# faverogian/diffusion-classifier

Hardware: AMD Instinct MI355X
Metric: images classified/sec (node), CIFAR-10 10-class x 50-step ELBO scoring (higher is better)
Workload: dtype bf16; 1 GPU; cifar10-unet-10x50; classes=10, trials=50, forwards_per_image=500, input=uniform [-1,1], parallelism=single

## Files before the change

### diffusion-classifier_amd/_lib.py

```python
import ctypes as C
import os

_HERE = os.path.dirname(os.path.abspath(__file__))
LIB_PATH = os.environ.get("DCAMD_LIB") or os.path.join(_HERE, "libdcamd.so")

ABI_VERSION = 4
DC_F32, DC_BF16, DC_F16 = 0, 1, 2
ACT_NONE, ACT_SILU, ACT_GEGLU, ACT_GELU_TANH = 0, 1, 2, 3
OP_QSAMPLE, OP_SINUSOID, OP_IGEMM, OP_GROUPNORM, OP_LAYERNORM, OP_ATTENTION, OP_EPS_MSE, OP_TBLOCK_FRONT = 1, 2, 3, 4, 5, 6, 7, 8

i32, i64, u64, f32, vp = C.c_int32, C.c_int64, C.c_uint64, C.c_float, C.c_void_p


class QsampleParams(C.Structure):
    _fields_ = [("x", vp), ("eps", vp), ("alpha", vp), ("sigma", vp), ("img_of_bj", vp),
                ("out", vp), ("out_dtype", i32),
                ("n_bj", i32), ("C", i32), ("H", i32), ("W", i32), ("ld", i32), ("im2col", i32), ("patch", i32)]


class SinusoidParams(C.Structure):
    _fields_ = [("lam", vp), ("out", vp), ("n", i32), ("dim", i32), ("flip_sin_to_cos", i32), ("freq_shift", f32)]


class IgemmParams(C.Structure):
# ... 39 lines not shown
    _fields_ = [("x", vp), ("Wp", vp), ("bp", vp), ("ln_g", vp), ("ln_b", vp), ("Wqkv", vp), ("Wo", vp), ("bo", vp),
                ("rowvec", vp), ("rowvec_map", vp), ("out", vp),
                ("dtype", i32), ("n", i32), ("L", i32), ("C", i32), ("heads", i32), ("ldx", i32), ("ld_out", i32), ("rowvec_ld", i32),
                ("ln_eps", f32), ("scale", f32)]


class EpsMseParams(C.Structure):
    _fields_ = [("pred", vp), ("eps", vp), ("x", vp), ("alpha", vp), ("sigma", vp),
                ("bj_of_unit", vp), ("img_of_bj", vp), ("out_index", vp),
                ("out", vp), ("n_units", i32), ("C", i32), ("H", i32), ("W", i32), ("ld", i32), ("v_param", i32), ("patch", i32)]


class DdpmStepParams(C.Structure):
    _fields_ = [("z", vp), ("pred", vp), ("noise", vp), ("out", vp),
                ("n", i32), ("C", i32), ("H", i32), ("W", i32), ("ld", i32), ("patch", i32), ("v_param", i32),
                ("w", f32), ("alpha_t", f32), ("sigma_t", f32), ("alpha_s", f32), ("c", f32), ("sd", f32), ("one_plus_w", f32)]


class Op(C.Structure):
    _fields_ = [("kind", i32), ("pad_", i32), ("params", vp)]


EXPORTS = ["dc_abi_version", "dc_last_error", "dc_arch", "dc_qsample", "dc_philox_normal", "dc_sinusoid",
           "dc_igemm", "dc_igemm_cout_pad", "dc_igemm_variant", "dc_igemm_gn_fusable", "dc_igemm_side_ok", "dc_igemm_ln_ok", "dc_igemm_qstats_parts", "dc_igemm_up4_ok", "dc_igemm_pn_ok", "dc_pn_timeouts", "dc_groupnorm", "dc_groupnorm_variant", "dc_groupnorm_ws_floats", "dc_groupnorm_splits",
           "dc_layernorm", "dc_layernorm_variant", "dc_attention", "dc_attention_variant", "dc_tblock_front", "dc_tblock_front_ok", "dc_eps_mse", "dc_ddpm_step", "dc_haar_dwt2", "dc_haar_idwt2", "dc_stage_topk", "dc_reduce_argmin", "dc_stage_maps", "dc_run_plan", "dc_run_plan_timed",
           "dc_packed_bytes", "dc_pack_weights_matrix", "dc_pack_weights_conv3x3", "dc_pack_weights_up4", "dc_pack_weights_geglu",
           "dc_fold_layernorm_bias", "dc_workspace_bytes_groupnorm", "dc_workspace_bytes_igemm", "dc_workspace_bytes_attention",
           "dc_workspace_bytes_layernorm"]

_lib = None


class DcamdError(RuntimeError):
    pass


def lib():
    global _lib
    if _lib is not None:
        return _lib
    if not os.path.exists(LIB_PATH):
        raise DcamdError(
            f"HIP extension {LIB_PATH} is missing — build it with `python -c 'import __graft_entry__ as g; g.build()'` "
            "(or `make -C diffusion-classifier_amd/csrc`). There is no CPU fallback for the scoring path.")
    L = C.CDLL(LIB_PATH)
    L.dc_abi_version.restype = i32
    L.dc_last_error.restype = C.c_char_p
# ... 19 lines not shown
                       ("dc_fold_layernorm_bias", [vp, vp, vp, i32, i32, vp, vp]),
                       ("dc_stage_topk", [vp, i32, i32, i32, i32, i32, vp, vp, vp]),
                       ("dc_reduce_argmin", [vp, i32, i32, i32, i32, vp, vp, vp]),
                       ("dc_stage_maps", [vp, i32, i32, i32, i32, i32, i32, i32, i32, i32, i32, i32, vp, vp])]:
        fn = getattr(L, name)
        fn.argtypes = argt
        fn.restype = i32
    L.dc_igemm_ln_ok.argtypes = [C.POINTER(IgemmParams)]
    L.dc_igemm_ln_ok.restype = C.c_int32
    L.dc_igemm_qstats_parts.argtypes = [C.POINTER(IgemmParams)]
    L.dc_igemm_qstats_parts.restype = C.c_int32
    L.dc_igemm_up4_ok.argtypes = [C.POINTER(IgemmParams)]
    L.dc_igemm_up4_ok.restype = C.c_int32
    L.dc_igemm_pn_ok.argtypes = [C.POINTER(IgemmParams)]
    L.dc_igemm_pn_ok.restype = C.c_int32
    L.dc_tblock_front_ok.argtypes = [C.POINTER(TblockFrontParams)]
    L.dc_tblock_front_ok.restype = C.c_int32
    L.dc_pn_timeouts.argtypes = []
    L.dc_pn_timeouts.restype = C.c_int32
    L.dc_igemm_side_ok.argtypes = [C.POINTER(IgemmParams)]
    L.dc_igemm_side_ok.restype = C.c_int32
    L.dc_igemm_variant.argtypes = [C.POINTER(IgemmParams)]
    L.dc_igemm_variant.restype = C.c_char_p
    L.dc_attention_variant.argtypes = [C.POINTER(AttentionParams)]
    L.dc_attention_variant.restype = C.c_char_p
    L.dc_groupnorm_variant.argtypes = [C.POINTER(GroupnormParams)]
    L.dc_groupnorm_variant.restype = C.c_char_p
    L.dc_layernorm_variant.argtypes = [C.POINTER(LayernormParams)]
    L.dc_layernorm_variant.restype = C.c_char_p
    L.dc_igemm_gn_fusable.argtypes = [C.POINTER(IgemmParams)]
    L.dc_igemm_gn_fusable.restype = i32
    L.dc_igemm_cout_pad.argtypes = [i32, i32]
    L.dc_igemm_cout_pad.restype = i32
    L.dc_packed_bytes.argtypes = [i32, i32, i32, i32]
    L.dc_packed_bytes.restype = i64
    for name, pt in (("dc_workspace_bytes_groupnorm", GroupnormParams), ("dc_workspace_bytes_igemm", IgemmParams),
                     ("dc_workspace_bytes_attention", AttentionParams), ("dc_workspace_bytes_layernorm", LayernormParams)):
        getattr(L, name).argtypes = [C.POINTER(pt)]
        getattr(L, name).restype = i64
    L.dc_groupnorm_ws_floats.argtypes = [i32, i32, i32]
    L.dc_groupnorm_ws_floats.restype = i64
    L.dc_groupnorm_splits.argtypes = [i32, i32, i32]
    L.dc_groupnorm_splits.restype = i32
    if L.dc_abi_version() != ABI_VERSION:
        raise DcamdError(f"libdcamd ABI {L.dc_abi_version()} != {ABI_VERSION} (stale libdcamd.so? rebuild with `make -C diffusion-classifier_amd/csrc`)")
    _lib = L
# ... 19 lines not shown
```

### diffusion-classifier_amd/csrc/igemm.hip

```cpp
#include <stdio.h>
#include <stdlib.h>
#include "conv3_halo.h"

template <typename T, int BM, int BN, int WGM, int WGN>
__global__ __launch_bounds__(256, 2) void igemm_kernel(const IgemmArgs a) {
  constexpr int EPC = Elem<T>::EPC;
  constexpr int BKE = 8 * EPC;
  constexpr int XL = BM / 32;
  constexpr int WL = (BN + 31) / 32;
  constexpr int WTM = BM / WGM, WTN = BN / WGN;
  constexpr int TM = WTM / 16, TN = WTN / 16;
  static_assert(WGM * WGN == 4, "4 waves");
  extern __shared__ __attribute__((aligned(16))) char smem[];
  constexpr int BUF = (BM + BN) * 128;

  const int t = threadIdx.x;
  const int lane = t & 63, wave = t >> 6;
  const int wm = wave / WGN, wn = wave % WGN;
  const int lr = lane & 15, lq = lane >> 4;

  int tile_m, tile_n;
  tile_of_block(a, tile_m, tile_n);

  const int HWo = a.Hout * a.Wout;
// ... 282 lines not shown
    case IG_PIPE: return dc_igemm_launch_pipe(a, p->dtype, c.shape, s);
    case IG_REG128: return dc_by_dtype(p->dtype, "dc_igemm: dtype", [&](auto t) { return launch<decltype(t), 128, 128, 2, 2>(a, s); });
    case IG_REG32: return dc_by_dtype(p->dtype, "dc_igemm: dtype", [&](auto t) { return launch<decltype(t), 128, 32, 4, 1>(a, s); });
  }
  return DC_ERR_ARG;
}

extern "C" int dc_igemm(const dc_igemm_params* p, dc_stream stream) {
  IgemmArgs a;
  const int rc = igemm_validate_and_fill(p, a);
  if (rc != DC_OK) return rc;
  const IgemmChoice c = igemm_choose(p, a);
  if (c.status != DC_OK) { dc_set_error("%s", c.message); return c.status; }
  return igemm_launch(c, a, p, stream);
}

extern "C" const char* dc_igemm_variant(const dc_igemm_params* p) {
  IgemmArgs a;
  if (igemm_validate_and_fill(p, a) != DC_OK) return "invalid";
  const IgemmChoice c = igemm_choose(p, a);
  return c.status == DC_OK ? igemm_name(c, p->dtype) : c.tag;
}

static int32_t igemm_accepts(const dc_igemm_params& q) {
  IgemmArgs a;
  return igemm_validate_and_fill(&q, a) == DC_OK && igemm_choose(&q, a).status == DC_OK ? 1 : 0;
}
alignas(16) static float g_probe_dummy[4] = {0.f, 0.f, 0.f, 0.f};

extern "C" int32_t dc_igemm_gn_fusable(const dc_igemm_params* p) {
  if (!p) return 0;
  dc_igemm_params q = *p;
  q.gn_scale = g_probe_dummy; q.gn_shift = g_probe_dummy;
  return igemm_accepts(q);
}

extern "C" int32_t dc_igemm_ln_ok(const dc_igemm_params* p) {
  if (!p) return 0;
  dc_igemm_params q = *p;
  if (!(q.ln_eps > 0.f)) q.ln_eps = 1e-5f;
  return igemm_accepts(q);
}

extern "C" int32_t dc_igemm_qstats_parts(const dc_igemm_params* p) {
  if (!p) return 0;
  dc_igemm_params q = *p;
// ... 35 lines not shown
```

### diffusion-classifier_amd/csrc/igemm_common.h

```cpp
#pragma once
#include "common.h"

struct IgemmArgs {
  const void* src0; const int32_t* map0; const void* src1; const int32_t* map1;
  const void* W; const float* bias;
  const float* rowvec; const int32_t* rowvec_map;
  const float* gate; const int32_t* gate_map;
  const void* residual; const int32_t* res_map;
  void* out;
  const float* gn_scale; const float* gn_shift; int gn_silu;
  const void* src2; const int32_t* map2; const void* W2; int C2, ld2;
  float ln_eps;
  float* qstats;
  void* pn_out; const float* pn_gamma; const float* pn_beta; unsigned* pn_cnt; int pn_ld, pn_groups, pn_silu; float pn_eps;
  int C0, C1, ld0, ld1, rowvec_ld, gate_ld, res_dtype, res_ld, out_dtype, out_ld, act;
  int taps, stride, upsample, Hin, Win, Hout, Wout, Cout;
  int M, Ktot, c0chunks, cpt, nk, tiles_m, tiles_n;
  int n_fast;
};

template <typename T> struct Mma;
template <> struct Mma<__bf16> {
  static __device__ __forceinline__ f32x4 run(const chunk16 w, const chunk16 x, f32x4 acc) {
    return __builtin_amdgcn_mfma_f32_16x16x32_bf16(__builtin_bit_cast(bf16x8, w), __builtin_bit_cast(bf16x8, x), acc, 0, 0, 0);
// ... 83 lines not shown
      }
      if (oc + 3 < cout_out && (a.out_ld & 3) == 0) {
        if (a.out_dtype == DC_F32) {
          *reinterpret_cast<float4*>(reinterpret_cast<float*>(a.out) + orow + oc) = make_float4(v[0], v[1], v[2], v[3]);
        } else if (a.out_dtype == DC_BF16) {
          __bf16 h[4] = {(__bf16)v[0], (__bf16)v[1], (__bf16)v[2], (__bf16)v[3]};
          *reinterpret_cast<uint2*>(reinterpret_cast<__bf16*>(a.out) + orow + oc) = *reinterpret_cast<uint2*>(h);
        } else {
          _Float16 h[4] = {(_Float16)v[0], (_Float16)v[1], (_Float16)v[2], (_Float16)v[3]};
          *reinterpret_cast<uint2*>(reinterpret_cast<_Float16*>(a.out) + orow + oc) = *reinterpret_cast<uint2*>(h);
        }
      } else {
#pragma unroll
        for (int r = 0; r < 4; ++r)
          if (oc + r < cout_out) store_as(a.out, orow + oc + r, a.out_dtype, v[r]);
      }
    }
  }
}

int dc_igemm_pipe_shape(const IgemmArgs& a);
int dc_igemm_launch_pipe(const IgemmArgs& a, int dtype, int shape, hipStream_t s);
int dc_igemm_launch_wide8(const IgemmArgs& a, int dtype, hipStream_t s);
__device__ __forceinline__ void tile_of_block_scalar(const IgemmArgs& a, int& tile_m, int& tile_n) {
  tile_of_block(a, tile_m, tile_n);
  tile_m = __builtin_amdgcn_readfirstlane(tile_m);
  tile_n = __builtin_amdgcn_readfirstlane(tile_n);
  asm volatile("" : "+s"(tile_m), "+s"(tile_n));
}

bool dc_conv3_halo_applicable(const IgemmArgs& a, int dtype);
int dc_conv3_halo_launch(const IgemmArgs& a, int dtype, int n_img, hipStream_t s);
bool dc_conv3_up4_applicable(const IgemmArgs& a, int dtype);
int dc_conv3_up4_launch(const IgemmArgs& a, int dtype, int n_img, hipStream_t s);
int dc_igemm_launch_pipe_up4(const IgemmArgs& a, int dtype, hipStream_t s);
bool dc_conv3_halo_pn_ok(const IgemmArgs& a, int dtype, bool up4);
unsigned dc_conv3_halo_pn_timeouts();
bool dc_conv3_ws_ok(const IgemmArgs& a, int dtype);
int dc_conv3_ws_launch(const IgemmArgs& a, int dtype, int n_img, hipStream_t s);
bool dc_igemm_xreg_applicable(const IgemmArgs& a, int dtype);
int dc_igemm_xreg_launch(const IgemmArgs& a, int dtype, hipStream_t s);
bool dc_conv3_thin_applicable(const IgemmArgs& a, int dtype);
int dc_conv3_thin_launch(const IgemmArgs& a, int dtype, int n_img, hipStream_t s);
```

### diffusion-classifier_amd/csrc/igemm_epilogue.h

```cpp
#pragma once
#include "igemm_common.h"
#ifndef DC_STAMP
#define DC_STAMP(k) do {} while (0)
#endif
#ifndef DC_HALO_ABL
#define DC_HALO_ABL() 0
#endif

__device__ __forceinline__ int epi_wrow(int R, bool geglu) {
  const int wn = R >> 6, i = (R >> 4) & 3, lq = (R >> 2) & 3, reg = R & 3;
  if (geglu) {
    const int o = wn * 32 + lq * 8 + (i >> 1) * 4 + reg;
    return (o >> 4) * 32 + ((i & 1) << 4) + (o & 15);
  }
  return wn * 64 + (i >> 1) * 32 + lq * 8 + (i & 1) * 4 + reg;
}

struct EpiRow { int o, r, samp; bool ok; };

__device__ __forceinline__ void ld8(const float* p, float (&v)[8]) {
  const f32x4 a = *reinterpret_cast<const f32x4*>(p), b = *reinterpret_cast<const f32x4*>(p + 4);
#pragma unroll
  for (int e = 0; e < 4; ++e) { v[e] = a[e]; v[4 + e] = b[e]; }
}

struct EpiNoPre { __device__ __forceinline__ void operator()() const {} };
struct EpiNoBias {
  static constexpr bool on = false, has_rowvec = false;
  __device__ __forceinline__ void operator()(int, float (&)[8], float (&)[8]) const {}
};

template <int V> struct EpiIC { static constexpr int value = V; };
struct EpiNoPnLocal { static constexpr bool on = false; static constexpr int IMG_FR = 4; };
struct EpiPnLocal8x8 { static constexpr bool on = true; static constexpr int IMG_FR = 4; };
struct EpiPnLocal4x4 { static constexpr bool on = true; static constexpr int IMG_FR = 1; };
struct EpiNoQs {
  static constexpr bool on = false;
  __device__ __forceinline__ bool operator()(int, int&, int&) const { return false; }
  __device__ __forceinline__ bool whole() const { return true; }
  __device__ __forceinline__ int parts() const { return 1; }
};

template <typename T, int TM, int ACT, bool GATE, bool TWO_SAMP, typename RowFn, typename PreFn = EpiNoPre, typename QsFn = EpiNoQs,
          typename BiasFn = EpiNoBias, typename PnL = EpiNoPnLocal>
__device__ __forceinline__ void epi_direct_act(const IgemmArgs& a, f32x4 (&acc)[4][TM], int tile_n, int wn, int lq,
                                               int samp_first, int samp_last, RowFn rowfn, PreFn prefn = PreFn(), QsFn qsfn = QsFn(),
                                               BiasFn biasfn = BiasFn(), PnL = PnL()) {
  static_assert(!PnL::on || (TM == 8 && ACT == DC_ACT_NONE && !GATE && (QsFn::on || PnL::IMG_FR == 1)), "wave-local GroupNorm: the plain 128-pixel halo epilogue");
  constexpr bool geglu = ACT == DC_ACT_GEGLU;
  constexpr int NK = geglu ? 1 : 2;
  constexpr int JB = TM;
  const int cout_out = geglu ? (a.Cout >> 1) : a.Cout;
  const int c0 = (geglu ? tile_n * 64 + wn * 32 : tile_n * 128 + wn * 64) + lq * 8;
  constexpr bool res16 = sizeof(T) == 2;
  bool con[NK];
#pragma unroll
  for (int k = 0; k < NK; ++k) con[k] = c0 + 32 * k < cout_out;

  {
    float bs[NK][8], bgt[8];
#pragma unroll
    for (int k = 0; k < NK; ++k) {
      const int c = c0 + 32 * k;
#pragma unroll
      for (int e = 0; e < 8; ++e) { bs[k][e] = 0.f; if (k == 0) bgt[e] = 0.f; }
      if constexpr (BiasFn::on) {
        biasfn(k, bs[k], bgt);
      } else if (a.bias && con[k]) {
        const int p = geglu ? (c >> 4) * 32 + (c & 15) : c;
        ld8(a.bias + p, bs[k]);
        if (geglu) ld8(a.bias + p + 16, bgt);
      }
    }
    const bool uni = samp_first == samp_last;
    prefn();
    const bool rv_uni = !BiasFn::has_rowvec && !geglu && a.rowvec && uni;
    float rvu[NK][8];
#pragma unroll
    for (int k = 0; k < NK; ++k)
#pragma unroll
      for (int e = 0; e < 8; ++e) rvu[k][e] = 0.f;
    if (rv_uni) {
#pragma unroll
      for (int k = 0; k < NK; ++k)
        if (con[k]) ld8(a.rowvec + (size_t)(a.rowvec_map ? a.rowvec_map[samp_first] : samp_first) * a.rowvec_ld + c0 + 32 * k, rvu[k]);
    }
#pragma unroll
    for (int j = 0; j < TM; ++j)
#pragma unroll
      for (int e = 0; e < 8; ++e) {
        if (geglu) { acc[(e >> 2) * 2][j][e & 3] += bs[0][e]; acc[(e >> 2) * 2 + 1][j][e & 3] += bgt[e]; }
        else {
#pragma unroll
          for (int k = 0; k < NK; ++k) acc[2 * k + (e >> 2)][j][e & 3] += bs[k][e];
        }
      }
    if (rv_uni) {
#pragma unroll
      for (int j = 0; j < TM; ++j)
#pragma unroll
        for (int e = 0; e < 8; ++e)
#pragma unroll
          for (int k = 0; k < NK; ++k) acc[2 * k + (e >> 2)][j][e & 3] += rvu[k][e];
    }
    if (!BiasFn::has_rowvec && !geglu && a.rowvec && !uni) {
      if (TWO_SAMP) {
#pragma unroll
        for (int k = 0; k < NK; ++k)
          if (con[k]) {
            float ra[8], rb[8];
            ld8(a.rowvec + (size_t)(a.rowvec_map ? a.rowvec_map[samp_first] : samp_first) * a.rowvec_ld + c0 + 32 * k, ra);
            ld8(a.rowvec + (size_t)(a.rowvec_map ? a.rowvec_map[samp_last] : samp_last) * a.rowvec_ld + c0 + 32 * k, rb);
#pragma unroll
            for (int j = 0; j < TM; ++j) {
              EpiRow rj;
              rowfn(j, rj);
              const bool second = rj.samp != samp_first;
#pragma unroll
              for (int e = 0; e < 8; ++e) acc[2 * k + (e >> 2)][j][e & 3] += second ? rb[e] : ra[e];
            }
          }
      } else {
#pragma unroll
        for (int j = 0; j < TM; ++j) {
          EpiRow rj;
          rowfn(j, rj);
#pragma unroll
          for (int k = 0; k < NK; ++k)
            if (con[k]) {
              float rv[8];
              ld8(a.rowvec + (size_t)(a.rowvec_map ? a.rowvec_map[rj.samp] : rj.samp) * a.rowvec_ld + c0 + 32 * k, rv);
#pragma unroll
              for (int e = 0; e < 8; ++e) acc[2 * k + (e >> 2)][j][e & 3] += rv[e];
            }
        }
      }
    }
  }

  DC_STAMP(3);
  int orow[TM];
#pragma unroll
  for (int j0 = 0; j0 < TM; j0 += JB) {
    EpiRow row[JB];
#pragma unroll
    for (int jj = 0; jj < JB; ++jj) { rowfn(j0 + jj, row[jj]); orow[j0 + jj] = row[jj].ok ? row[jj].o : -1; }
    chunk16 rc[JB][NK];
#pragma unroll
    for (int jj = 0; jj < JB; ++jj)
#pragma unroll
      for (int k = 0; k < NK; ++k) {
        rc[jj][k] = chunk16{0u, 0u, 0u, 0u};
        if (res16 && a.residual && row[jj].ok && con[k])
          rc[jj][k] = *reinterpret_cast<const chunk16*>(reinterpret_cast<const char*>(a.residual) + ((size_t)row[jj].r * a.res_ld + c0 + 32 * k) * 2);
      }
    if (j0 == 0) DC_STAMP(4);
#pragma unroll
    for (int jj = 0; jj < JB; ++jj) {
      const int j = j0 + jj;
#pragma unroll
      for (int k = 0; k < NK; ++k) {
        if (!(row[jj].ok && con[k])) continue;
        float rf[8], gt[8];
#pragma unroll
        for (int e = 0; e < 8; ++e) { rf[e] = 0.f; gt[e] = 1.f; }
        if (GATE) ld8(a.gate + (size_t)(a.gate_map ? a.gate_map[row[jj].samp] : row[jj].samp) * a.gate_ld + c0 + 32 * k, gt);
        if (a.residual) {
          if (!res16) ld8(reinterpret_cast<const float*>(a.residual) + (size_t)row[jj].r * a.res_ld + c0 + 32 * k, rf);
          else chunk_to_f<T>(rc[jj][k], rf);
        }
#pragma unroll
        for (int e = 0; e < 8; ++e) {
          if (geglu) {
            acc[(e >> 2) * 2][j][e & 3] = acc[(e >> 2) * 2][j][e & 3] * gelu_erf_t<T>(acc[(e >> 2) * 2 + 1][j][e & 3]) + rf[e];
          } else {
            float x = acc[2 * k + (e >> 2)][j][e & 3];
            if (ACT == DC_ACT_SILU) x = silu_t<T>(x);
            if (ACT == DC_ACT_GELU_TANH) x = gelu_tanh_t<T>(x);
            if (GATE) x *= gt[e];
            acc[2 * k + (e >> 2)][j][e & 3] = x + rf[e];
          }
        }
      }
    }
  }
  DC_STAMP(5);
  float pnr[(PnL::on && PnL::IMG_FR == 4) ? 2 : 1][NK][4];
  float pgm[PnL::on ? NK : 1][8], pbt[PnL::on ? NK : 1][8];
  if constexpr (PnL::on) {
#pragma unroll
// ... 47 lines not shown
            r[k][2 * qd] = __builtin_fmaf(S, inv_n, piv[k][qd]);
            r[k][2 * qd + 1] = fmaxf(__builtin_fmaf(-S * S, inv_n, Q), 0.f);
          }
        if constexpr (PnL::on && PnL::IMG_FR == 4) {
#pragma unroll
          for (int k = 0; k < NK; ++k)
#pragma unroll
            for (int e = 0; e < 4; ++e) pnr[h][k][e] = r[k][e];
        }
        int n = 0, part = 0;
        if ((threadIdx.x & 15) == 0 && qsfn(h, n, part)) {
#pragma unroll
          for (int k = 0; k < NK; ++k)
            if (con[k])
              *reinterpret_cast<f32x4*>(a.qstats + (((size_t)n * qsfn.parts() + part) * (a.Cout >> 2) + ((c0 + 32 * k) >> 2)) * 2) =
                  f32x4{r[k][0], r[k][1], r[k][2], r[k][3]};
        }
      };
      if (qsfn.whole()) emit(EpiIC<0>{}, EpiIC<TM>{}, 0);
      else { emit(EpiIC<0>{}, EpiIC<TM / 2>{}, 0); emit(EpiIC<TM / 2>{}, EpiIC<TM>{}, 1); }
    }
  }
  auto store_all = [&](void* outp, int ld, int odt) {
    if (odt == DC_F32) {
#pragma unroll
      for (int j = 0; j < TM; ++j)
#pragma unroll
        for (int k = 0; k < NK; ++k)
          if (orow[j] >= 0 && con[k]) {
            float* op = reinterpret_cast<float*>(outp) + (size_t)orow[j] * ld + c0 + 32 * k;
            if (geglu) { *reinterpret_cast<f32x4*>(op) = acc[0][j]; *reinterpret_cast<f32x4*>(op + 4) = acc[2][j]; }
            else { *reinterpret_cast<f32x4*>(op) = acc[2 * k][j]; *reinterpret_cast<f32x4*>(op + 4) = acc[2 * k + 1][j]; }
          }
    } else {
#pragma unroll
      for (int j = 0; j < TM; ++j)
#pragma unroll
        for (int k = 0; k < NK; ++k)
          if (orow[j] >= 0 && con[k]) {
            float v[8];
#pragma unroll
            for (int e = 0; e < 8; ++e) v[e] = geglu ? acc[(e >> 2) * 2][j][e & 3] : acc[2 * k + (e >> 2)][j][e & 3];
            *reinterpret_cast<chunk16*>(reinterpret_cast<T*>(outp) + (size_t)orow[j] * ld + c0 + 32 * k) = f_to_chunk<T>(v);
          }
    }
  };
  if constexpr (!PnL::on) {
    store_all(a.out, a.out_ld, a.out_dtype);
  } else {
    if (a.out) store_all(a.out, a.out_ld, a.out_dtype);
    constexpr int IFR = PnL::IMG_FR, NIMG = TM / IFR;
    const int qpg = (a.Cout / a.pn_groups) >> 2;
    const float nq = (float)(IFR * 64);
#pragma unroll
    for (int h = 0; h < NIMG; ++h) {
#pragma unroll
      for (int k = 0; k < NK; ++k) {
        float rq[4];
        if constexpr (IFR == 4) {
#pragma unroll
          for (int e = 0; e < 4; ++e) rq[e] = pnr[h][k][e];
        } else {
#pragma clang fp contract(off)
          auto share0l = [](float v) { return __builtin_bit_cast(float, __builtin_amdgcn_update_dpp(0, __builtin_bit_cast(int, v), 0x150, 0xF, 0xF, true)); };
          auto row_suml = [](float v) {
            v += __builtin_bit_cast(float, __builtin_amdgcn_update_dpp(0, __builtin_bit_cast(int, v), 0xB1, 0xF, 0xF, true));
            v += __builtin_bit_cast(float, __builtin_amdgcn_update_dpp(0, __builtin_bit_cast(int, v), 0x4E, 0xF, 0xF, true));
            v += __builtin_bit_cast(float, __builtin_amdgcn_update_dpp(0, __builtin_bit_cast(int, v), 0x141, 0xF, 0xF, true));
            v += __builtin_bit_cast(float, __builtin_amdgcn_update_dpp(0, __builtin_bit_cast(int, v), 0x140, 0xF, 0xF, true));
            return v;
          };
// ... 59 lines not shown
        if (a.pn_silu) {
#pragma unroll
          for (int jj = 0; jj < IFR; ++jj)
#pragma unroll
            for (int e = 0; e < 8; ++e) {
              const float x = acc[2 * k + (e >> 2)][h * IFR + jj][e & 3];
              acc[2 * k + (e >> 2)][h * IFR + jj][e & 3] = silu_t<T>(x * ga[e] + gb[e]);
            }
        } else {
#pragma unroll
          for (int jj = 0; jj < IFR; ++jj)
#pragma unroll
            for (int e = 0; e < 8; ++e) {
              const float x = acc[2 * k + (e >> 2)][h * IFR + jj][e & 3];
              acc[2 * k + (e >> 2)][h * IFR + jj][e & 3] = x * ga[e] + gb[e];
            }
        }
      }
    }
    store_all(a.pn_out, a.pn_ld, sizeof(T) == 4 ? DC_F32 : (int)a.out_dtype);
  }
}

template <typename T, int TM, typename RowFn>
__device__ __forceinline__ void epi_direct(const IgemmArgs& a, f32x4 (&acc)[4][TM], int tile_n, int wn, int lq,
                                           int samp_first, int samp_last, RowFn rowfn) {
  switch (a.act) {
    case DC_ACT_SILU: epi_direct_act<T, TM, DC_ACT_SILU, false, false>(a, acc, tile_n, wn, lq, samp_first, samp_last, rowfn); break;
    case DC_ACT_GEGLU: epi_direct_act<T, TM, DC_ACT_GEGLU, false, false>(a, acc, tile_n, wn, lq, samp_first, samp_last, rowfn); break;
    case DC_ACT_GELU_TANH: epi_direct_act<T, TM, DC_ACT_GELU_TANH, false, false>(a, acc, tile_n, wn, lq, samp_first, samp_last, rowfn); break;
    default:
      if (a.gate) epi_direct_act<T, TM, DC_ACT_NONE, true, false>(a, acc, tile_n, wn, lq, samp_first, samp_last, rowfn);
      else epi_direct_act<T, TM, DC_ACT_NONE, false, false>(a, acc, tile_n, wn, lq, samp_first, samp_last, rowfn);
      break;
  }
}
```

### diffusion-classifier_amd/csrc/igemm_wide.hip

```cpp
#include <stdlib.h>
#include "igemm_epilogue.h"

static __device__ chunk16 g_zero_page_w[16];
DC_CLOCK_DECL(igemm_wide)

typedef const __attribute__((address_space(1))) void* gptr_t;
typedef __attribute__((address_space(3))) void* lptr_t;

template <typename T, int EV>
__global__ __launch_bounds__(512, 2) void igemm_wide8_kernel(const IgemmArgs a) {
  constexpr int EPC = Elem<T>::EPC;
  constexpr int BKE = 8 * EPC;
  constexpr int HALF = 128 * 128;
  constexpr int BUF = 4 * HALF;
  constexpr int SX0 = 0, SW0 = HALF, SX1 = 2 * HALF, SW1 = 3 * HALF;
  extern __shared__ __attribute__((aligned(16))) char smem[];

  const int t = threadIdx.x;
  const int lane = t & 63;
  const int wave = __builtin_amdgcn_readfirstlane(t >> 6);
  const int wm = wave >> 1, wn = wave & 1;
  const int lr = lane & 15, lq = lane >> 4;
  int tile_m, tile_n;
  tile_of_block(a, tile_m, tile_n);
  const int HWo = a.Hout * a.Wout;
  const int nk = a.nk, c0chunks = a.c0chunks;

  const int lchunk = (t & 7) ^ ((t >> 4) & 7);
  const T* xr0[2][2]; const T* xr1[2][2];
  int wro[2][2];
#pragma unroll
  for (int i = 0; i < 2; ++i) {
    const int hr = 64 * i + (t >> 3);
#pragma unroll
    for (int xh = 0; xh < 2; ++xh) {
      const int m = tile_m * 256 + (hr >> 5) * 64 + xh * 32 + (hr & 31);
      const bool vm = m < a.M;
      const int mm = vm ? m : 0;
      const int n = mm / HWo;
      const int rem = mm - n * HWo;
      const int n0 = a.map0 ? a.map0[n] : n;
      const int n1 = a.src1 ? (a.map1 ? a.map1[n] : n) : 0;
      const T* b0 = reinterpret_cast<const T*>(a.src0) + ((size_t)n0 * HWo + rem) * a.ld0 + lchunk * EPC;
      const T* b1 = reinterpret_cast<const T*>(a.src1) + ((size_t)n1 * HWo + rem) * a.ld1 + lchunk * EPC;
      xr0[xh][i] = vm ? b0 : nullptr;
      xr1[xh][i] = (vm && a.src1) ? b1 : nullptr;
      asm volatile("" ::"v"(xr0[xh][i]), "v"(xr1[xh][i]));
// ... 57 lines not shown
  _Pragma("unroll") for (int sub = 0; sub < 2; ++sub)                                                         \
    _Pragma("unroll") for (int jj = 0; jj < 2; ++jj)                                                          \
      _Pragma("unroll") for (int i = 0; i < 4; ++i)                                                           \
        acc[H][i][J0 + jj] = Mma<T>::run(wf[sub][i], XF[sub][jj], acc[H][i][J0 + jj]);                        \
  __builtin_amdgcn_s_setprio(0);                                                                              \
  __builtin_amdgcn_sched_barrier(0);
#define W8_READ_X(DST, SLOT)                                                                                \
  _Pragma("unroll") for (int sub = 0; sub < 2; ++sub) {                                                       \
    DST[sub][0] = ds_read16_async_off<SLOT>(xfo[sub] + bufo);                                                 \
    DST[sub][1] = ds_read16_async_off<SLOT + 2048>(xfo[sub] + bufo);                                          \
  }
#define W8_READ_W(SLOT)                                                                                     \
  _Pragma("unroll") for (int sub = 0; sub < 2; ++sub) {                                                       \
    wf[sub][0] = ds_read16_async_off<SLOT>(wfo[sub] + bufo);                                                  \
    wf[sub][1] = ds_read16_async_off<SLOT + 2048>(wfo[sub] + bufo);                                           \
    wf[sub][2] = ds_read16_async_off<SLOT + 4096>(wfo[sub] + bufo);                                           \
    wf[sub][3] = ds_read16_async_off<SLOT + 6144>(wfo[sub] + bufo);                                           \
  }
#define W8_WAIT_W() asm volatile("s_waitcnt lgkmcnt(0)" : "+v"(wf[0][0]), "+v"(wf[0][1]), "+v"(wf[0][2]), "+v"(wf[0][3]), \
                                 "+v"(wf[1][0]), "+v"(wf[1][1]), "+v"(wf[1][2]), "+v"(wf[1][3]))
#define W8_WAIT_X(XF) asm volatile("s_waitcnt lgkmcnt(0)" : "+v"(XF[0][0]), "+v"(XF[0][1]), "+v"(XF[1][0]), "+v"(XF[1][1]))

  DC_CLOCK(0);
  for (int kt = 0; kt < nk; ++kt) {
    const uint32_t bufo = (uint32_t)(kt & 1) * BUF;
    lgkm_fence0();
    W8_READ_X(xa, SX0)
    __builtin_amdgcn_sched_barrier(0);
    W8_READ_W(SW0)
    stage_w(kt + 1, 1, SW1);
    asm volatile("s_waitcnt lgkmcnt(8)" : "+v"(xa[0][0]), "+v"(xa[0][1]), "+v"(xa[1][0]), "+v"(xa[1][1]));
    __builtin_amdgcn_s_barrier();
    W8_WAIT_W();
    W8_MMA(0, xa, 0)
    __builtin_amdgcn_s_barrier();
    W8_READ_X(xb, SX1)
    stage_x(kt + 2, 0, SX0);
    __builtin_amdgcn_s_barrier();
    W8_WAIT_X(xb);
    W8_MMA(0, xb, 2)
    __builtin_amdgcn_s_barrier();
    W8_READ_W(SW1)
    stage_w(kt + 2, 0, SW0);
    __builtin_amdgcn_s_barrier();
    W8_WAIT_W();
    W8_MMA(1, xb, 2)
    __builtin_amdgcn_s_barrier();
    stage_x(kt + 2, 1, SX1);
    if (kt + 2 < nk) asm volatile("s_waitcnt vmcnt(6)" ::: "memory");
    else asm volatile("s_waitcnt vmcnt(0)" ::: "memory");
    __builtin_amdgcn_s_barrier();
    W8_MMA(1, xa, 0)
    __builtin_amdgcn_s_barrier();
  }
#undef W8_MMA
#undef W8_READ_X
#undef W8_READ_W
#undef W8_WAIT_W
#undef W8_WAIT_X
  DC_CLOCK(1);
  if (wave < 4) __builtin_amdgcn_s_barrier();

  const int mw0 = tile_m * 256 + wm * 64;
  auto rowfn = [&](int j, EpiRow& r) {
    const int m = mw0 + j * 16 + lr;
    r.ok = m < a.M;
    const int mm = r.ok ? m : a.M - 1;
    const int n = mm / HWo;
    r.samp = n;
    r.o = mm;
    r.r = (a.residual && a.res_map) ? a.res_map[n] * HWo + (mm - n * HWo) : mm;
  };
  const int sf = min(mw0, a.M - 1) / HWo, sl = min(mw0 + 63, a.M - 1) / HWo;
  constexpr int ACT = EV == 3 ? DC_ACT_GELU_TANH : (EV == 2 ? DC_ACT_GEGLU : DC_ACT_NONE);
  epi_direct_act<T, 4, ACT, EV == 4, false>(a, acc[0], tile_n * 2 + wn, 0, lq, sf, sl, rowfn);
  __builtin_amdgcn_sched_barrier(0);
  epi_direct_act<T, 4, ACT, EV == 4, false>(a, acc[1], tile_n * 2 + wn, 1, lq, sf, sl, rowfn);
}

template <typename T, int EV>
static int launch_wide8(const IgemmArgs& a0, hipStream_t s) {
  constexpr int lds = 2 * 4 * 128 * 128;
  static bool attr_done = false;
  auto kern = igemm_wide8_kernel<T, EV>;
  if (!attr_done) {
    (void)hipFuncSetAttribute(reinterpret_cast<const void*>(kern), hipFuncAttributeMaxDynamicSharedMemorySize, lds);
    attr_done = true;
  }
  IgemmArgs a = a0;
  a.tiles_m = (a.M + 255) / 256;
  a.tiles_n = a0.tiles_n / 2;
  const long long nblk = (long long)a.tiles_m * a.tiles_n;
  if (nblk <= 0 || nblk > 0x7fffffffLL) { dc_set_error("dc_igemm: bad grid %lld", nblk); return DC_ERR_SHAPE; }
  if ((long long)a0.tiles_n * 128 * a.Ktot >= (1LL << 31)) { dc_set_error("dc_igemm(wide8): weight matrix of %d x %d too large", a0.tiles_n * 128, a.Ktot); return DC_ERR_SHAPE; }
  hipLaunchKernelGGL(kern, dim3((unsigned)nblk), dim3(512), lds, s, a);
  return dc_check_launch("dc_igemm(wide8)");
}

template <typename T>
static int launch_wide8_t(const IgemmArgs& a, hipStream_t s) {
  if (a.act == DC_ACT_GELU_TANH) return launch_wide8<T, 3>(a, s);
  if (a.act == DC_ACT_GEGLU) return launch_wide8<T, 2>(a, s);
  if (a.gate) return launch_wide8<T, 4>(a, s);
  return launch_wide8<T, 0>(a, s);
}

int dc_igemm_launch_wide8(const IgemmArgs& a, int dtype, hipStream_t s) {
  return dc_by_dtype(dtype, "dc_igemm: dtype", [&](auto t) { return launch_wide8_t<decltype(t)>(a, s); });
}
```

### include/dcamd.h

```cpp
#ifndef DCAMD_H
#define DCAMD_H

#include <stddef.h>
#include <stdint.h>

#ifdef __cplusplus
extern "C" {
#endif

#define DC_ABI_VERSION 4

typedef void* dc_stream;

typedef enum { DC_OK = 0, DC_ERR_ARG = -1, DC_ERR_SHAPE = -2, DC_ERR_DTYPE = -3,
               DC_ERR_ALIGN = -4, DC_ERR_LAUNCH = -5, DC_ERR_UNSUPPORTED = -6 } dc_status;

typedef enum { DC_F32 = 0, DC_BF16 = 1, DC_F16 = 2 } dc_dtype;

typedef enum { DC_ACT_NONE = 0, DC_ACT_SILU = 1, DC_ACT_GEGLU = 2, DC_ACT_GELU_TANH = 3 } dc_act;

int dc_abi_version(void);
const char* dc_last_error(void);
const char* dc_arch(void);

// ... 13 lines not shown

typedef struct {
  int32_t dtype, taps, stride, upsample;
  int32_t n_img, Hin, Win, Hout, Wout;
  const void* src0; const int32_t* map0; int32_t C0, ld0;
  const void* src1; const int32_t* map1; int32_t C1, ld1;
  const void* W; int32_t Cout, tile_n;
  const float* bias;
  const float* rowvec; const int32_t* rowvec_map; int32_t rowvec_ld, act;
  const float* gate; const int32_t* gate_map; int32_t gate_ld, pad2_;
  const void* residual; const int32_t* res_map; int32_t res_dtype, res_ld;
  void* out; int32_t out_dtype, out_ld;
  const float* gn_scale; const float* gn_shift; int32_t gn_silu, pad3_;
  const void* src2; const int32_t* map2; const void* W2; int32_t C2, ld2;
  float ln_eps;
  int32_t up4;
  float* qstats;
  void* pn_out; const float* pn_gamma; const float* pn_beta; uint32_t* pn_cnt;
  int32_t pn_ld, pn_groups, pn_silu; float pn_eps;
} dc_igemm_params;
int dc_igemm(const dc_igemm_params* p, dc_stream s);
int32_t dc_igemm_cout_pad(int32_t cout, int32_t tile_n);
const char* dc_igemm_variant(const dc_igemm_params* p);
int32_t dc_igemm_gn_fusable(const dc_igemm_params* p);
int32_t dc_igemm_side_ok(const dc_igemm_params* p);
int32_t dc_igemm_ln_ok(const dc_igemm_params* p);
int32_t dc_igemm_qstats_parts(const dc_igemm_params* p);
int32_t dc_igemm_pn_ok(const dc_igemm_params* p);
int32_t dc_pn_timeouts(void);
int32_t dc_igemm_up4_ok(const dc_igemm_params* p);

int64_t dc_packed_bytes(int32_t cout, int32_t K, int32_t dtype, int32_t tile_n);
int dc_pack_weights_matrix(const float* w, int32_t cout, int32_t K, int32_t kpad, const int32_t* row_perm, const float* col_scale,
                           void* out, int32_t dtype, int32_t tile_n, dc_stream s);
int dc_pack_weights_conv3x3(const float* w, int32_t cout, int32_t cin, int32_t c_lo, int32_t c_hi, int32_t kpad, void* out,
                            int32_t dtype, int32_t tile_n, dc_stream s);
int dc_pack_weights_up4(const float* w, int32_t cout, int32_t cin, void* out, int32_t dtype, int32_t tile_n, dc_stream s);
int dc_pack_weights_geglu(const float* w, const float* bias, int32_t n_half, int32_t K, const float* ln_gamma, const float* ln_beta,
                          void* out_w, float* out_bias, int32_t* perm_ws, int32_t dtype, dc_stream s);
int dc_fold_layernorm_bias(const float* w, const float* bias, const float* ln_beta, int32_t cout, int32_t K, float* out_bias, dc_stream s);

typedef struct {
  const void* x; const int32_t* map0;
  const void* x1; const int32_t* map1;
  void* y; int32_t dtype, out_dtype;
  int32_t n, HW, C, C1, groups, silu, splits; float eps;
// ... 76 lines not shown
```

Measured before the change: 227.2 images/s.

## Specialise wide8 igemm epilogue per side-operand set with maskless full-tile path

Adds compile-time epilogue specialisations for the 16-bit wide8 implicit-GEMM kernel, keyed on which of bias, rowvec and residual are present. Full tiles take a maskless store and residual-load path with scalar base rows. The block-to-tile mapping is also changed to group consecutive tiles per XCD. The aim is to cut runtime pointer checks, bounds masks and address arithmetic in the epilogue, and to improve L2 locality across XCDs. The cost is more template instances and code size, and the new XCD remap could change cache behaviour for other shapes.

Measured after the change: 228.2 images/s (median of 6 runs). No clear change (+0.4%).

```diff
diff --git a/diffusion-classifier_amd/_lib.py b/diffusion-classifier_amd/_lib.py
--- a/diffusion-classifier_amd/_lib.py
+++ b/diffusion-classifier_amd/_lib.py
@@ -85,7 +85,7 @@
 
 
 EXPORTS = ["dc_abi_version", "dc_last_error", "dc_arch", "dc_qsample", "dc_philox_normal", "dc_sinusoid",
-           "dc_igemm", "dc_igemm_cout_pad", "dc_igemm_variant", "dc_igemm_gn_fusable", "dc_igemm_side_ok", "dc_igemm_ln_ok", "dc_igemm_qstats_parts", "dc_igemm_up4_ok", "dc_igemm_pn_ok", "dc_pn_timeouts", "dc_groupnorm", "dc_groupnorm_variant", "dc_groupnorm_ws_floats", "dc_groupnorm_splits",
+           "dc_igemm", "dc_igemm_cout_pad", "dc_igemm_variant", "dc_igemm_epilogue_instance", "dc_igemm_gn_fusable", "dc_igemm_side_ok", "dc_igemm_ln_ok", "dc_igemm_qstats_parts", "dc_igemm_up4_ok", "dc_igemm_pn_ok", "dc_pn_timeouts", "dc_groupnorm", "dc_groupnorm_variant", "dc_groupnorm_ws_floats", "dc_groupnorm_splits",
            "dc_layernorm", "dc_layernorm_variant", "dc_attention", "dc_attention_variant", "dc_tblock_front", "dc_tblock_front_ok", "dc_eps_mse", "dc_ddpm_step", "dc_haar_dwt2", "dc_haar_idwt2", "dc_stage_topk", "dc_reduce_argmin", "dc_stage_maps", "dc_run_plan", "dc_run_plan_timed",
            "dc_packed_bytes", "dc_pack_weights_matrix", "dc_pack_weights_conv3x3", "dc_pack_weights_up4", "dc_pack_weights_geglu",
            "dc_fold_layernorm_bias", "dc_workspace_bytes_groupnorm", "dc_workspace_bytes_igemm", "dc_workspace_bytes_attention",
@@ -151,6 +151,8 @@
     L.dc_igemm_side_ok.restype = C.c_int32
     L.dc_igemm_variant.argtypes = [C.POINTER(IgemmParams)]
     L.dc_igemm_variant.restype = C.c_char_p
+    L.dc_igemm_epilogue_instance.argtypes = [C.POINTER(IgemmParams)]
+    L.dc_igemm_epilogue_instance.restype = C.c_char_p
     L.dc_attention_variant.argtypes = [C.POINTER(AttentionParams)]
     L.dc_attention_variant.restype = C.c_char_p
     L.dc_groupnorm_variant.argtypes = [C.POINTER(GroupnormParams)]
diff --git a/diffusion-classifier_amd/csrc/igemm.hip b/diffusion-classifier_amd/csrc/igemm.hip
--- a/diffusion-classifier_amd/csrc/igemm.hip
+++ b/diffusion-classifier_amd/csrc/igemm.hip
@@ -328,6 +328,14 @@
   return c.status == DC_OK ? igemm_name(c, p->dtype) : c.tag;
 }
 
+extern "C" const char* dc_igemm_epilogue_instance(const dc_igemm_params* p) {
+  IgemmArgs a;
+  if (igemm_validate_and_fill(p, a) != DC_OK) return "invalid";
+  const IgemmChoice c = igemm_choose(p, a);
+  if (c.status != DC_OK) return c.tag;
+  return (c.kernel == IG_PIPE && c.shape == 2) ? dc_igemm_wide8_instance(a, p->dtype) : "generic";
+}
+
 static int32_t igemm_accepts(const dc_igemm_params& q) {
   IgemmArgs a;
   return igemm_validate_and_fill(&q, a) == DC_OK && igemm_choose(&q, a).status == DC_OK ? 1 : 0;
diff --git a/diffusion-classifier_amd/csrc/igemm_common.h b/diffusion-classifier_amd/csrc/igemm_common.h
--- a/diffusion-classifier_amd/csrc/igemm_common.h
+++ b/diffusion-classifier_amd/csrc/igemm_common.h
@@ -129,6 +129,7 @@
 int dc_igemm_pipe_shape(const IgemmArgs& a);
 int dc_igemm_launch_pipe(const IgemmArgs& a, int dtype, int shape, hipStream_t s);
 int dc_igemm_launch_wide8(const IgemmArgs& a, int dtype, hipStream_t s);
+const char* dc_igemm_wide8_instance(const IgemmArgs& a, int dtype);
 __device__ __forceinline__ void tile_of_block_scalar(const IgemmArgs& a, int& tile_m, int& tile_n) {
   tile_of_block(a, tile_m, tile_n);
   tile_m = __builtin_amdgcn_readfirstlane(tile_m);
diff --git a/diffusion-classifier_amd/csrc/igemm_epilogue.h b/diffusion-classifier_amd/csrc/igemm_epilogue.h
--- a/diffusion-classifier_amd/csrc/igemm_epilogue.h
+++ b/diffusion-classifier_amd/csrc/igemm_epilogue.h
@@ -41,12 +41,22 @@
   __device__ __forceinline__ int parts() const { return 1; }
 };
 
+
+struct EpiGeneric { static constexpr bool known = false, bias = false, rowvec = false, residual = false, res_map = false; };
+template <bool BIAS, bool ROWVEC, bool RES, bool RESMAP> struct EpiSpec {
+  static_assert(RES || !RESMAP, "res_map without a residual");
+  static constexpr bool known = true, bias = BIAS, rowvec = ROWVEC, residual = RES, res_map = RESMAP;
+};
+
 template <typename T, int TM, int ACT, bool GATE, bool TWO_SAMP, typename RowFn, typename PreFn = EpiNoPre, typename QsFn = EpiNoQs,
-          typename BiasFn = EpiNoBias, typename PnL = EpiNoPnLocal>
+          typename BiasFn = EpiNoBias, typename PnL = EpiNoPnLocal, typename Spec = EpiGeneric, bool FULL = false>
 __device__ __forceinline__ void epi_direct_act(const IgemmArgs& a, f32x4 (&acc)[4][TM], int tile_n, int wn, int lq,
                                                int samp_first, int samp_last, RowFn rowfn, PreFn prefn = PreFn(), QsFn qsfn = QsFn(),
-                                               BiasFn biasfn = BiasFn(), PnL = PnL()) {
+                                               BiasFn biasfn = BiasFn(), PnL = PnL(), Spec = Spec()) {
   static_assert(!PnL::on || (TM == 8 && ACT == DC_ACT_NONE && !GATE && (QsFn::on || PnL::IMG_FR == 1)), "wave-local GroupNorm: the plain 128-pixel halo epilogue");
+  static_assert(!Spec::known || (!QsFn::on && !PnL::on && !BiasFn::on), "specialised epilogue: plain side operands only");
+  static_assert(!FULL || Spec::known, "the maskless form belongs to the specialised instances");
+#define EPI_HAS(ptr, flag) (Spec::known ? Spec::flag : ((ptr) != nullptr))
   constexpr bool geglu = ACT == DC_ACT_GEGLU;
   constexpr int NK = geglu ? 1 : 2;
   constexpr int JB = TM;
@@ -55,7 +65,7 @@
   constexpr bool res16 = sizeof(T) == 2;
   bool con[NK];
 #pragma unroll
-  for (int k = 0; k < NK; ++k) con[k] = c0 + 32 * k < cout_out;
+  for (int k = 0; k < NK; ++k) con[k] = FULL ? true : c0 + 32 * k < cout_out;
 
   {
     float bs[NK][8], bgt[8];
@@ -66,15 +76,15 @@
       for (int e = 0; e < 8; ++e) { bs[k][e] = 0.f; if (k == 0) bgt[e] = 0.f; }
       if constexpr (BiasFn::on) {
         biasfn(k, bs[k], bgt);
-      } else if (a.bias && con[k]) {
+      } else if (EPI_HAS(a.bias, bias) && con[k]) {
         const int p = geglu ? (c >> 4) * 32 + (c & 15) : c;
         ld8(a.bias + p, bs[k]);
         if (geglu) ld8(a.bias + p + 16, bgt);
       }
     }
-    const bool uni = samp_first == samp_last;
+    const bool uni = FULL ? true : samp_first == samp_last;
     prefn();
-    const bool rv_uni = !BiasFn::has_rowvec && !geglu && a.rowvec && uni;
+    const bool rv_uni = !BiasFn::has_rowvec && !geglu && EPI_HAS(a.rowvec, rowvec) && uni;
     float rvu[NK][8];
 #pragma unroll
     for (int k = 0; k < NK; ++k)
@@ -103,7 +113,7 @@
 #pragma unroll
           for (int k = 0; k < NK; ++k) acc[2 * k + (e >> 2)][j][e & 3] += rvu[k][e];
     }
-    if (!BiasFn::has_rowvec && !geglu && a.rowvec && !uni) {
+    if (!BiasFn::has_rowvec && !geglu && EPI_HAS(a.rowvec, rowvec) && !uni) {
       if (TWO_SAMP) {
 #pragma unroll
         for (int k = 0; k < NK; ++k)
@@ -140,18 +150,34 @@
 
   DC_STAMP(3);
   int orow[TM];
+  int brow = 0, drow = 0;
+  if constexpr (FULL) {
+    EpiRow r0;
+    rowfn(0, r0);
+    brow = __builtin_amdgcn_readfirstlane(r0.o);
+    drow = r0.o - brow;
+  }
 #pragma unroll
   for (int j0 = 0; j0 < TM; j0 += JB) {
     EpiRow row[JB];
 #pragma unroll
-    for (int jj = 0; jj < JB; ++jj) { rowfn(j0 + jj, row[jj]); orow[j0 + jj] = row[jj].ok ? row[jj].o : -1; }
+    for (int jj = 0; jj < JB; ++jj) {
+      rowfn(j0 + jj, row[jj]);
+      if (FULL) row[jj].ok = true;
+      orow[j0 + jj] = row[jj].ok ? row[jj].o : -1;
+    }
     chunk16 rc[JB][NK];
 #pragma unroll
     for (int jj = 0; jj < JB; ++jj)
 #pragma unroll
       for (int k = 0; k < NK; ++k) {
         rc[jj][k] = chunk16{0u, 0u, 0u, 0u};
-        if (res16 && a.residual && row[jj].ok && con[k])
+        if constexpr (FULL && !Spec::res_map) {
+          if (res16 && EPI_HAS(a.residual, residual)) {
+            const char* rb = reinterpret_cast<const char*>(a.residual) + (size_t)(brow + 16 * (j0 + jj)) * a.res_ld * 2;
+            rc[jj][k] = *reinterpret_cast<const chunk16*>(rb + (uint32_t)((drow * a.res_ld + c0) * 2) + 64 * k);
+          }
+        } else if (res16 && EPI_HAS(a.residual, residual) && row[jj].ok && con[k])
           rc[jj][k] = *reinterpret_cast<const chunk16*>(reinterpret_cast<const char*>(a.residual) + ((size_t)row[jj].r * a.res_ld + c0 + 32 * k) * 2);
       }
     if (j0 == 0) DC_STAMP(4);
@@ -165,7 +191,7 @@
 #pragma unroll
         for (int e = 0; e < 8; ++e) { rf[e] = 0.f; gt[e] = 1.f; }
         if (GATE) ld8(a.gate + (size_t)(a.gate_map ? a.gate_map[row[jj].samp] : row[jj].samp) * a.gate_ld + c0 + 32 * k, gt);
-        if (a.residual) {
+        if (EPI_HAS(a.residual, residual)) {
           if (!res16) ld8(reinterpret_cast<const float*>(a.residual) + (size_t)row[jj].r * a.res_ld + c0 + 32 * k, rf);
           else chunk_to_f<T>(rc[jj][k], rf);
         }
@@ -259,7 +285,25 @@
     }
   }
   auto store_all = [&](void* outp, int ld, int odt) {
-    if (odt == DC_F32) {
+    if constexpr (FULL) {
+      const uint32_t lo = (uint32_t)(drow * ld + c0);
+#pragma unroll
+      for (int j = 0; j < TM; ++j) {
+        T* ob = reinterpret_cast<T*>(outp) + (size_t)(brow + 16 * j) * ld;
+#pragma unroll
+        for (int k = 0; k < NK; ++k) {
+          if constexpr (sizeof(T) == 4) {
+            *reinterpret_cast<f32x4*>(ob + lo + 32 * k) = acc[geglu ? 0 : 2 * k][j];
+            *reinterpret_cast<f32x4*>(ob + lo + 32 * k + 4) = acc[geglu ? 2 : 2 * k + 1][j];
+          } else {
+            float v[8];
+#pragma unroll
+            for (int e = 0; e < 8; ++e) v[e] = geglu ? acc[(e >> 2) * 2][j][e & 3] : acc[2 * k + (e >> 2)][j][e & 3];
+            *reinterpret_cast<chunk16*>(ob + lo + 32 * k) = f_to_chunk<T>(v);
+          }
+        }
+      }
+    } else if (odt == DC_F32) {
 #pragma unroll
       for (int j = 0; j < TM; ++j)
 #pragma unroll
@@ -283,7 +327,7 @@
     }
   };
   if constexpr (!PnL::on) {
-    store_all(a.out, a.out_ld, a.out_dtype);
+    store_all(a.out, a.out_ld, Spec::known ? (sizeof(T) == 4 ? DC_F32 : DC_BF16) : a.out_dtype);
   } else {
     if (a.out) store_all(a.out, a.out_ld, a.out_dtype);
     constexpr int IFR = PnL::IMG_FR, NIMG = TM / IFR;
@@ -389,6 +433,8 @@
   }
 }
 
+#undef EPI_HAS
+
 template <typename T, int TM, typename RowFn>
 __device__ __forceinline__ void epi_direct(const IgemmArgs& a, f32x4 (&acc)[4][TM], int tile_n, int wn, int lq,
                                            int samp_first, int samp_last, RowFn rowfn) {
diff --git a/diffusion-classifier_amd/csrc/igemm_wide.hip b/diffusion-classifier_amd/csrc/igemm_wide.hip
--- a/diffusion-classifier_amd/csrc/igemm_wide.hip
+++ b/diffusion-classifier_amd/csrc/igemm_wide.hip
@@ -3,12 +3,24 @@
 
 static __device__ chunk16 g_zero_page_w[16];
 DC_CLOCK_DECL(igemm_wide)
+#ifdef DC_W8_STAMPS
+static __device__ unsigned long long* g_w8_stamps;
+extern "C" void dc_debug_set_w8_stamps(unsigned long long* p) { (void)hipMemcpyToSymbol(HIP_SYMBOL(g_w8_stamps), &p, sizeof(p)); }
+#define W8_STAMP(v) do { __builtin_amdgcn_sched_barrier(0); v = __builtin_amdgcn_s_memtime(); __builtin_amdgcn_sched_barrier(0); } while (0)
+#else
+#define W8_STAMP(v) do {} while (0)
+#endif
 
 typedef const __attribute__((address_space(1))) void* gptr_t;
 typedef __attribute__((address_space(3))) void* lptr_t;
 
-template <typename T, int EV>
+template <typename T, int EV, typename Spec = EpiGeneric>
 __global__ __launch_bounds__(512, 2) void igemm_wide8_kernel(const IgemmArgs a) {
+  static_assert(!Spec::known || (EV == 0 && sizeof(T) == 2), "specialised epilogues: the plain variant of the 16-bit types");
+#ifdef DC_W8_STAMPS
+  unsigned long long w8_t0 = 0, w8_t1 = 0, w8_t2 = 0, w8_t3 = 0;
+#endif
+  W8_STAMP(w8_t0);
   constexpr int EPC = Elem<T>::EPC;
   constexpr int BKE = 8 * EPC;
   constexpr int HALF = 128 * 128;
@@ -22,7 +34,15 @@
   const int wm = wave >> 1, wn = wave & 1;
   const int lr = lane & 15, lq = lane >> 4;
   int tile_m, tile_n;
-  tile_of_block(a, tile_m, tile_n);
+  {
+    const int nblk = gridDim.x, bid = blockIdx.x;
+    const int q8 = nblk >> 3, r8 = nblk & 7, xcd = bid & 7;
+    const int lid = (xcd < r8 ? xcd * (q8 + 1) : r8 * (q8 + 1) + (xcd - r8) * q8) + (bid >> 3);
+    const int inner = a.n_fast ? a.tiles_n : a.tiles_m;
+    const int outer_i = lid / inner, inner_i = lid - outer_i * inner;
+    tile_m = a.n_fast ? outer_i : inner_i;
+    tile_n = a.n_fast ? inner_i : outer_i;
+  }
   const int HWo = a.Hout * a.Wout;
   const int nk = a.nk, c0chunks = a.c0chunks;
 
@@ -126,6 +146,7 @@
 #define W8_WAIT_X(XF) asm volatile("s_waitcnt lgkmcnt(0)" : "+v"(XF[0][0]), "+v"(XF[0][1]), "+v"(XF[1][0]), "+v"(XF[1][1]))
 
   DC_CLOCK(0);
+  W8_STAMP(w8_t1);
   for (int kt = 0; kt < nk; ++kt) {
     const uint32_t bufo = (uint32_t)(kt & 1) * BUF;
     lgkm_fence0();
@@ -163,6 +184,7 @@
 #undef W8_WAIT_W
 #undef W8_WAIT_X
   DC_CLOCK(1);
+  W8_STAMP(w8_t2);
   if (wave < 4) __builtin_amdgcn_s_barrier();
 
   const int mw0 = tile_m * 256 + wm * 64;
@@ -173,20 +195,42 @@
     const int n = mm / HWo;
     r.samp = n;
     r.o = mm;
-    r.r = (a.residual && a.res_map) ? a.res_map[n] * HWo + (mm - n * HWo) : mm;
+    const bool mapped = Spec::known ? Spec::res_map : (a.residual && a.res_map);
+    r.r = mapped ? a.res_map[n] * HWo + (mm - n * HWo) : mm;
   };
-  const int sf = min(mw0, a.M - 1) / HWo, sl = min(mw0 + 63, a.M - 1) / HWo;
   constexpr int ACT = EV == 3 ? DC_ACT_GELU_TANH : (EV == 2 ? DC_ACT_GEGLU : DC_ACT_NONE);
-  epi_direct_act<T, 4, ACT, EV == 4, false>(a, acc[0], tile_n * 2 + wn, 0, lq, sf, sl, rowfn);
-  __builtin_amdgcn_sched_barrier(0);
-  epi_direct_act<T, 4, ACT, EV == 4, false>(a, acc[1], tile_n * 2 + wn, 1, lq, sf, sl, rowfn);
-}
-
-template <typename T, int EV>
+  int sf = 0, sl = 0;
+  if (!Spec::known || Spec::rowvec) { sf = min(mw0, a.M - 1) / HWo; sl = min(mw0 + 63, a.M - 1) / HWo; }
+  if constexpr (Spec::known) {
+    const bool full = __builtin_amdgcn_readfirstlane((mw0 + 64 <= a.M && (tile_n * 2 + wn + 1) * 128 <= a.Cout && sf == sl) ? 1 : 0) != 0;
+    if (full) {
+      epi_direct_act<T, 4, ACT, false, false, decltype(rowfn), EpiNoPre, EpiNoQs, EpiNoBias, EpiNoPnLocal, Spec, true>(a, acc[0], tile_n * 2 + wn, 0, lq, sf, sl, rowfn);
+      __builtin_amdgcn_sched_barrier(0);
+      epi_direct_act<T, 4, ACT, false, false, decltype(rowfn), EpiNoPre, EpiNoQs, EpiNoBias, EpiNoPnLocal, Spec, true>(a, acc[1], tile_n * 2 + wn, 1, lq, sf, sl, rowfn);
+    } else {
+      epi_direct_act<T, 4, ACT, false, false, decltype(rowfn), EpiNoPre, EpiNoQs, EpiNoBias, EpiNoPnLocal, Spec, false>(a, acc[0], tile_n * 2 + wn, 0, lq, sf, sl, rowfn);
+      __builtin_amdgcn_sched_barrier(0);
+      epi_direct_act<T, 4, ACT, false, false, decltype(rowfn), EpiNoPre, EpiNoQs, EpiNoBias, EpiNoPnLocal, Spec, false>(a, acc[1], tile_n * 2 + wn, 1, lq, sf, sl, rowfn);
+    }
+  } else {
+    epi_direct_act<T, 4, ACT, EV == 4, false>(a, acc[0], tile_n * 2 + wn, 0, lq, sf, sl, rowfn);
+    __builtin_amdgcn_sched_barrier(0);
+    epi_direct_act<T, 4, ACT, EV == 4, false>(a, acc[1], tile_n * 2 + wn, 1, lq, sf, sl, rowfn);
+  }
+#ifdef DC_W8_STAMPS
+  W8_STAMP(w8_t3);
+  if (threadIdx.x == 0 && g_w8_stamps) {
+    g_w8_stamps[blockIdx.x * 4] = w8_t1 - w8_t0; g_w8_stamps[blockIdx.x * 4 + 1] = w8_t2 - w8_t1;
+    g_w8_stamps[blockIdx.x * 4 + 2] = w8_t3 - w8_t2; g_w8_stamps[blockIdx.x * 4 + 3] = w8_t3 - w8_t0;
+  }
+#endif
+}
+
+template <typename T, int EV, typename Spec = EpiGeneric>
 static int launch_wide8(const IgemmArgs& a0, hipStream_t s) {
   constexpr int lds = 2 * 4 * 128 * 128;
   static bool attr_done = false;
-  auto kern = igemm_wide8_kernel<T, EV>;
+  auto kern = igemm_wide8_kernel<T, EV, Spec>;
   if (!attr_done) {
     (void)hipFuncSetAttribute(reinterpret_cast<const void*>(kern), hipFuncAttributeMaxDynamicSharedMemorySize, lds);
     attr_done = true;
@@ -201,14 +245,42 @@
   return dc_check_launch("dc_igemm(wide8)");
 }
 
+enum { W8_GENERIC = 0, W8_NONE, W8_BIAS, W8_BIAS_RES, W8_BIAS_RV_RES, W8_N_INST };
+static const char* const w8_inst_name[W8_N_INST] = {"generic", "wide8:plain", "wide8:bias", "wide8:bias+residual", "wide8:bias+rowvec+residual"};
+
+static int wide8_instance(const IgemmArgs& a, int dtype) {
+  static const bool generic = getenv("DCAMD_EPI_GENERIC") != nullptr;
+  if (generic || dtype == DC_F32 || a.act != DC_ACT_NONE || a.gate || a.out_dtype != dtype || a.qstats) return W8_GENERIC;
+  if (a.out_ld >= (1 << 20) || (a.residual && (a.res_ld >= (1 << 20) || a.res_map))) return W8_GENERIC;
+  const int key = (a.bias ? 1 : 0) | (a.rowvec ? 2 : 0) | (a.residual ? 4 : 0);
+  switch (key) {
+    case 0: return W8_NONE;
+    case 1: return W8_BIAS;
+    case 5: return W8_BIAS_RES;
+    case 7: return W8_BIAS_RV_RES;
+    default: return W8_GENERIC;
+  }
+}
+
 template <typename T>
-static int launch_wide8_t(const IgemmArgs& a, hipStream_t s) {
+static int launch_wide8_t(const IgemmArgs& a, int dtype, hipStream_t s) {
   if (a.act == DC_ACT_GELU_TANH) return launch_wide8<T, 3>(a, s);
   if (a.act == DC_ACT_GEGLU) return launch_wide8<T, 2>(a, s);
   if (a.gate) return launch_wide8<T, 4>(a, s);
+  if constexpr (sizeof(T) == 2) {
+    switch (wide8_instance(a, dtype)) {
+      case W8_NONE: return launch_wide8<T, 0, EpiSpec<false, false, false, false>>(a, s);
+      case W8_BIAS: return launch_wide8<T, 0, EpiSpec<true, false, false, false>>(a, s);
+      case W8_BIAS_RES: return launch_wide8<T, 0, EpiSpec<true, false, true, false>>(a, s);
+      case W8_BIAS_RV_RES: return launch_wide8<T, 0, EpiSpec<true, true, true, false>>(a, s);
+      default: break;
+    }
+  }
   return launch_wide8<T, 0>(a, s);
 }
 
+const char* dc_igemm_wide8_instance(const IgemmArgs& a, int dtype) { return w8_inst_name[wide8_instance(a, dtype)]; }
+
 int dc_igemm_launch_wide8(const IgemmArgs& a, int dtype, hipStream_t s) {
-  return dc_by_dtype(dtype, "dc_igemm: dtype", [&](auto t) { return launch_wide8_t<decltype(t)>(a, s); });
-}
+  return dc_by_dtype(dtype, "dc_igemm: dtype", [&](auto t) { return launch_wide8_t<decltype(t)>(a, dtype, s); });
+}
diff --git a/include/dcamd.h b/include/dcamd.h
--- a/include/dcamd.h
+++ b/include/dcamd.h
@@ -59,6 +59,7 @@
 int dc_igemm(const dc_igemm_params* p, dc_stream s);
 int32_t dc_igemm_cout_pad(int32_t cout, int32_t tile_n);
 const char* dc_igemm_variant(const dc_igemm_params* p);
+const char* dc_igemm_epilogue_instance(const dc_igemm_params* p);
 int32_t dc_igemm_gn_fusable(const dc_igemm_params* p);
 int32_t dc_igemm_side_ok(const dc_igemm_params* p);
 int32_t dc_igemm_ln_ok(const dc_igemm_params* p);
```
